# shivangchopra11/MedMoE

Measured on AMD Instinct MI355X. Metric: image-text pairs/sec at global batch 1024, higher is better.
Workload: dtype bf16; 1 GPU; cfg2: ViT-B/16 + 12-layer text tower (frozen), 8 experts top-2, 224x224x3 + 77 tokens, fwd+bwd+clip+Adam; global_batch=1024, per_gpu_batch=1024, parallelism=dp1

## Files before the change

### medmoe_amd/csrc/attention.hip

```cpp
#include "common.h"
#include "options.h"

#define HD 64

__device__ __forceinline__ int tpos(int r) {
  const int o = r & 31;
  return (r & ~31) + (((o & 15) >> 2) << 3) + ((o >> 4) << 2) + (o & 3);
}

template <int CNT, int RT>
__device__ __forceinline__ void fill_rowmajor(char* lds, const bf16_t* src, long long row_stride, int n_valid, int tid) {
  constexpr int PER = (CNT + RT - 1) / RT;
  uint4 v[PER];
#pragma unroll
  for (int i = 0; i < PER; ++i) {
    const int idx = min(tid + i * RT, CNT - 1);
    const int row = idx >> 3, c = idx & 7;
    v[i] = *(const uint4*)(src + (long long)min(row, n_valid - 1) * row_stride + c * 8);
  }
#pragma unroll
  for (int i = 0; i < PER; ++i) {
    const int idx = tid + i * RT;
    const int row = idx >> 3, c = idx & 7;
    if (idx < CNT) *(uint4*)(lds + row * 128 + ((c ^ (row & 7)) << 4)) = v[i];
  }
}

__device__ __forceinline__ void fill_transposed(char* lds, const bf16_t* src, long long row_stride, int n_valid,
                                                int stride_bytes, int tid) {
  for (int i = tid; i < (64 * stride_bytes) / 16; i += 256) *(uint4*)(lds + i * 16) = make_uint4(0, 0, 0, 0);
  __syncthreads();
  for (int idx = tid; idx < n_valid * 8; idx += 256) {
    const int row = idx >> 3, c = idx & 7;
    const uint4 v = *(const uint4*)(src + (long long)row * row_stride + c * 8);
    const uint32_t w[4] = {v.x, v.y, v.z, v.w};
    const int pos = tpos(row);
#pragma unroll
    for (int e = 0; e < 4; ++e) {
      *(bf16_t*)(lds + (c * 8 + 2 * e) * stride_bytes + pos * 2) = (bf16_t)(w[e] & 0xffff);
      *(bf16_t*)(lds + (c * 8 + 2 * e + 1) * stride_bytes + pos * 2) = (bf16_t)(w[e] >> 16);
    }
  }
}

__device__ __forceinline__ bf16x8_t tr_frag(const char* img, int row0, int col0, int lane) {
  const int q = (lane & 15) >> 2, pp = lane & 3;
  const int ra = row0 + 4 * (lane >> 4) + q, rb = ra + 16;
  const int col = col0 + 4 * pp;
  const int ch = col >> 3, within = (col & 7) << 1;
  const bf16x4_t lo = __builtin_amdgcn_ds_read_tr16_b64_v4bf16(
      (__attribute__((address_space(3))) bf16x4_t*)(img + ra * 128 + ((ch ^ (ra & 7)) << 4) + within));
  const bf16x4_t hi = __builtin_amdgcn_ds_read_tr16_b64_v4bf16(
      (__attribute__((address_space(3))) bf16x4_t*)(img + rb * 128 + ((ch ^ (rb & 7)) << 4) + within));
  return __builtin_shufflevector(lo, hi, 0, 1, 2, 3, 4, 5, 6, 7);
}

__device__ __forceinline__ bf16x8_t load_frag_global(const bf16_t* base, long long row_stride, int row, int chunk) {
  const uint4 v = *(const uint4*)(base + (long long)row * row_stride + chunk * 8);
  return __builtin_bit_cast(bf16x8_t, v);
}

__device__ __forceinline__ bf16x8_t pack_frag(const f32x4_t& a, const f32x4_t& b) {
  uint4 v;
  v.x = pack2bf(a[0], a[1]); v.y = pack2bf(a[2], a[3]);
  v.z = pack2bf(b[0], b[1]); v.w = pack2bf(b[2], b[3]);
  return __builtin_bit_cast(bf16x8_t, v);
}

template <int NKT>
struct AttnGeom {
  static constexpr int NKP = NKT * 16;
  static constexpr int KS = (NKT + 1) / 2;
  static constexpr int RMROWS = KS * 32;
  static constexpr int RM_BYTES = RMROWS * 128;
  static constexpr int FILL = RMROWS * 8;
};

#ifdef ATTN_TIMING
__device__ unsigned long long g_attn_timing[8];
#define ATTN_T(...) __VA_ARGS__
#else
#define ATTN_T(...)
#endif

template <int NKT, bool MASKED, int RT>
__global__ __launch_bounds__(RT, RT == 256 ? 2 : 4) void attn_fwd_kernel(const bf16_t* __restrict__ qkv, bf16_t* __restrict__ out,
                                                         float* __restrict__ lse, const unsigned char* __restrict__ key_mask,
                                                         int Nmax, int H, float scale, const int* __restrict__ seq_off) {
  using G = AttnGeom<NKT>;
  constexpr int CH = 8;
  constexpr int NCH = (NKT + CH - 1) / CH;
  __shared__ __attribute__((aligned(16))) char smem[2 * G::RM_BYTES + G::NKP * 4];
  char* sK = smem;
  char* sV = smem + G::RM_BYTES;
  float* sMask = (float*)(smem + 2 * G::RM_BYTES);
  const int tid = threadIdx.x, lane = tid & 63, wid = tid >> 6;
  const int b = blockIdx.x / H, h = blockIdx.x - b * H;
  const int D = H * HD;
  const long long rs = 3LL * D;
  const long long row0 = seq_off ? (long long)seq_off[b] : (long long)b * Nmax;
  const int N = seq_off ? max(1, min(seq_off[b + 1] - seq_off[b], Nmax)) : Nmax;
  const bf16_t* base = qkv + row0 * rs + h * HD;

  fill_rowmajor<G::FILL, RT>(sK, base + D, rs, N, tid);
  fill_rowmajor<G::FILL, RT>(sV, base + 2 * D, rs, N, tid);
  for (int k = tid; k < G::NKP; k += RT)
    sMask[k] = (k < N && (!key_mask || key_mask[(long long)b * Nmax + k])) ? 0.f : -INFINITY;
  __syncthreads();

  const int fr = lane & 15, g = lane >> 4;
  const int nqb = (N + 15) >> 4;
  const float c2 = scale * 1.44269504088896f;
  bf16x8_t qf[2], qn[2];
  {
    const int qc0 = min(wid * 16 + fr, N - 1);
    qf[0] = load_frag_global(base, rs, qc0, g);
    qf[1] = load_frag_global(base, rs, qc0, 4 + g);
  }
  for (int qb = wid; qb < nqb; qb += RT / 64) {
    const int q = qb * 16 + fr;
    {
      const int qcn = min((qb + RT / 64) * 16 + fr, N - 1);
      qn[0] = load_frag_global(base, rs, qcn, g);
      qn[1] = load_frag_global(base, rs, qcn, 4 + g);
    }
    float m = -INFINITY, lp = 0.f;
    f32x4_t o[4];
#pragma unroll
    for (int nd = 0; nd < 4; ++nd) o[nd] = (f32x4_t){0.f, 0.f, 0.f, 0.f};
#pragma unroll 1
    for (int c = 0; c < NCH; ++c) {
      const int kt0 = c * CH;
      f32x4_t s[CH];
#pragma unroll
      for (int u = 0; u < CH; ++u) {
        s[u] = (f32x4_t){0.f, 0.f, 0.f, 0.f};
        if (kt0 + u < NKT) {
          const char* kr = sK + ((kt0 + u) * 16 + fr) * 128;
#pragma unroll
          for (int ks = 0; ks < 2; ++ks) {
            const bf16x8_t kf = *(const bf16x8_t*)(kr + (((ks * 4 + g) ^ (fr & 7)) << 4));
            s[u] = __builtin_amdgcn_mfma_f32_16x16x32_bf16(kf, qf[ks], s[u], 0, 0, 0);
          }
        }
      }
      float alpha;
      f32x2_t l2 = {0.f, 0.f};
      if constexpr (MASKED) {
        float bm = -INFINITY;
#pragma unroll
        for (int u = 0; u < CH; ++u)
          if (kt0 + u < NKT) {
            const float4 mk = *(const float4*)(sMask + (kt0 + u) * 16 + g * 4);
            const f32x2_t t0 = (f32x2_t){s[u][0], s[u][1]} * c2 + (f32x2_t){mk.x, mk.y};
            const f32x2_t t1 = (f32x2_t){s[u][2], s[u][3]} * c2 + (f32x2_t){mk.z, mk.w};
            s[u][0] = t0[0]; s[u][1] = t0[1]; s[u][2] = t1[0]; s[u][3] = t1[1];
            bm = fmaxf(fmaxf(bm, fmaxf(t0[0], t0[1])), fmaxf(t1[0], t1[1]));
          }
        bm = fmaxf(bm, __shfl_xor(bm, 16, 64));
        bm = fmaxf(bm, __shfl_xor(bm, 32, 64));
        const float mn = fmaxf(m, bm);
        const float ms = (mn == -INFINITY) ? 0.f : mn;
        alpha = __builtin_amdgcn_exp2f(m - ms);
        m = mn;
#pragma unroll
        for (int u = 0; u < CH; ++u)
          if (kt0 + u < NKT) {
            const f32x2_t d0 = (f32x2_t){s[u][0], s[u][1]} - ms, d1 = (f32x2_t){s[u][2], s[u][3]} - ms;
            const f32x2_t e0 = {__builtin_amdgcn_exp2f(d0[0]), __builtin_amdgcn_exp2f(d0[1])};
            const f32x2_t e1 = {__builtin_amdgcn_exp2f(d1[0]), __builtin_amdgcn_exp2f(d1[1])};
            s[u][0] = e0[0]; s[u][1] = e0[1]; s[u][2] = e1[0]; s[u][3] = e1[1];
            l2 += e0 + e1;
          }
      } else {
        float bm = fmaxf(fmaxf(s[0][0], s[0][1]), fmaxf(s[0][2], s[0][3]));
#pragma unroll
        for (int u = 1; u < CH; ++u)
          if (kt0 + u < NKT) bm = fmaxf(fmaxf(bm, fmaxf(s[u][0], s[u][1])), fmaxf(s[u][2], s[u][3]));
        bm = fmaxf(bm, __shfl_xor(bm, 16, 64));
        bm = fmaxf(bm, __shfl_xor(bm, 32, 64));
        const float mn = fmaxf(m, bm * c2);
        alpha = __builtin_amdgcn_exp2f(m - mn);
        m = mn;
        const float nm = -mn;
#pragma unroll
        for (int u = 0; u < CH; ++u)
          if (kt0 + u < NKT) {
            const f32x2_t d0 = (f32x2_t){s[u][0], s[u][1]} * c2 + nm, d1 = (f32x2_t){s[u][2], s[u][3]} * c2 + nm;
            f32x2_t e0 = {__builtin_amdgcn_exp2f(d0[0]), __builtin_amdgcn_exp2f(d0[1])};
            f32x2_t e1 = {__builtin_amdgcn_exp2f(d1[0]), __builtin_amdgcn_exp2f(d1[1])};
            if ((kt0 + u) * 16 + 16 > N) {
              const int k0 = (kt0 + u) * 16 + g * 4;
              e0[0] = k0 < N ? e0[0] : 0.f; e0[1] = k0 + 1 < N ? e0[1] : 0.f;
              e1[0] = k0 + 2 < N ? e1[0] : 0.f; e1[1] = k0 + 3 < N ? e1[1] : 0.f;
            }
            s[u][0] = e0[0]; s[u][1] = e0[1]; s[u][2] = e1[0]; s[u][3] = e1[1];
            l2 += e0 + e1;
          }
      }
      lp = lp * alpha + l2[0] + l2[1];
#pragma unroll
      for (int nd = 0; nd < 4; ++nd) {
        if (c > 0) o[nd] *= alpha;
#pragma unroll
        for (int t = 0; t < CH / 2; ++t)
          if (kt0 + 2 * t < NKT) {
            const bf16x8_t pf = pack_frag(s[2 * t], s[2 * t + 1]);
            const bf16x8_t vf = tr_frag(sV, (kt0 + 2 * t) * 16, nd * 16, lane);
            o[nd] = __builtin_amdgcn_mfma_f32_16x16x32_bf16(vf, pf, o[nd], 0, 0, 0);
          }
      }
    }
    float l = lp;
    l += __shfl_xor(l, 16, 64);
    l += __shfl_xor(l, 32, 64);
    const float inv = l > 0.f ? 1.f / l : 0.f;
    if (q < N) {
      if (g == 0) lse[((long long)b * H + h) * Nmax + q] = (m + __log2f(l)) * 0.693147180559945f;
#pragma unroll
      for (int nd = 0; nd < 4; ++nd) {
        const f32x4_t v = o[nd] * inv;
        uint2 pk; pk.x = pack2bf(v[0], v[1]); pk.y = pack2bf(v[2], v[3]);
        *(uint2*)(out + (row0 + q) * D + h * HD + nd * 16 + g * 4) = pk;
      }
    }
    qf[0] = qn[0]; qf[1] = qn[1];
  }
}

template <int NKT, bool MASKED, int RT>
__global__ __launch_bounds__(RT, 4) void attn_bwd_dq_kernel(const bf16_t* __restrict__ qkv, const bf16_t* __restrict__ o,
                                                          const bf16_t* __restrict__ dout, const float* __restrict__ lse,
                                                          const unsigned char* __restrict__ key_mask,
                                                          bf16_t* __restrict__ dqkv, float* __restrict__ delta,
                                                          int Nmax, int H, float scale, const int* __restrict__ seq_off) {
  using G = AttnGeom<NKT>;
  __shared__ __attribute__((aligned(16))) char smem[2 * G::RM_BYTES + G::NKP * 4];
  char* sK = smem;
  char* sV = smem + G::RM_BYTES;
  float* sMask = (float*)(smem + 2 * G::RM_BYTES);
  const int tid = threadIdx.x, lane = tid & 63, wid = tid >> 6;
  const int b = blockIdx.x / H, h = blockIdx.x - b * H;
  const int D = H * HD;
  const long long rs = 3LL * D;
  const long long row0 = seq_off ? (long long)seq_off[b] : (long long)b * Nmax;
  const int N = seq_off ? max(1, min(seq_off[b + 1] - seq_off[b], Nmax)) : Nmax;
  const bf16_t* base = qkv + row0 * rs + h * HD;
  const bf16_t* obase = o + row0 * D + h * HD;
  const bf16_t* dobase = dout + row0 * D + h * HD;

  fill_rowmajor<G::FILL, RT>(sK, base + D, rs, N, tid);
  fill_rowmajor<G::FILL, RT>(sV, base + 2 * D, rs, N, tid);
  for (int k = tid; k < G::NKP; k += RT)
    sMask[k] = (k < N && (!key_mask || key_mask[(long long)b * Nmax + k])) ? 0.f : -INFINITY;
  __syncthreads();

  const int fr = lane & 15, g = lane >> 4;
  const int nqb = (N + 15) >> 4;
  bf16x8_t qf[2], dof[2], of[2], qn[2], don[2], on[2];
  {
    const int qc0 = min(wid * 16 + fr, N - 1);
#pragma unroll
    for (int ks = 0; ks < 2; ++ks) {
      qf[ks] = load_frag_global(base, rs, qc0, ks * 4 + g);
      dof[ks] = load_frag_global(dobase, D, qc0, ks * 4 + g);
      of[ks] = load_frag_global(obase, D, qc0, ks * 4 + g);
    }
  }
  for (int qb = wid; qb < nqb; qb += RT / 64) {
    const int q = qb * 16 + fr;
    const int qc = min(q, N - 1);
    {
      const int qcn = min((qb + RT / 64) * 16 + fr, N - 1);
#pragma unroll
      for (int ks = 0; ks < 2; ++ks) {
        qn[ks] = load_frag_global(base, rs, qcn, ks * 4 + g);
        don[ks] = load_frag_global(dobase, D, qcn, ks * 4 + g);
        on[ks] = load_frag_global(obase, D, qcn, ks * 4 + g);
      }
    }
    float dl = 0.f;
#pragma unroll
    for (int ks = 0; ks < 2; ++ks)
#pragma unroll
      for (int e = 0; e < 8; ++e) dl += (float)dof[ks][e] * (float)of[ks][e];
    dl += __shfl_xor(dl, 16, 64);
    dl += __shfl_xor(dl, 32, 64);
    const float c2 = scale * 1.44269504088896f;
    const float nL2 = -lse[((long long)b * H + h) * Nmax + qc] * 1.44269504088896f;
    if (g == 0 && q < N) delta[((long long)b * H + h) * Nmax + q] = dl;

    f32x4_t acc[4];
#pragma unroll
    for (int nd = 0; nd < 4; ++nd) acc[nd] = (f32x4_t){0.f, 0.f, 0.f, 0.f};
#pragma unroll 1
    for (int t = 0; t < G::KS; ++t) {
      f32x4_t ds[2];
#pragma unroll
      for (int u = 0; u < 2; ++u) {
        const int kt = 2 * t + u;
        ds[u] = (f32x4_t){0.f, 0.f, 0.f, 0.f};
        if (kt < NKT) {
          f32x4_t s = {0.f, 0.f, 0.f, 0.f}, dp = {0.f, 0.f, 0.f, 0.f};
          const char* kr = sK + (kt * 16 + fr) * 128;
          const char* vr = sV + (kt * 16 + fr) * 128;
#pragma unroll
          for (int ks = 0; ks < 2; ++ks) {
            const int off = ((ks * 4 + g) ^ (fr & 7)) << 4;
            s = __builtin_amdgcn_mfma_f32_16x16x32_bf16(*(const bf16x8_t*)(kr + off), qf[ks], s, 0, 0, 0);
            dp = __builtin_amdgcn_mfma_f32_16x16x32_bf16(*(const bf16x8_t*)(vr + off), dof[ks], dp, 0, 0, 0);
          }
          if (MASKED || kt * 16 + 16 > N) {
            const float4 mk = *(const float4*)(sMask + kt * 16 + g * 4);
            const float mkv[4] = {mk.x, mk.y, mk.z, mk.w};
#pragma unroll
            for (int r = 0; r < 4; ++r) ds[u][r] = __builtin_amdgcn_exp2f(s[r] * c2 + (mkv[r] + nL2)) * (dp[r] - dl);
          } else {
            const f32x2_t t0 = (f32x2_t){s[0], s[1]} * c2 + nL2, t1 = (f32x2_t){s[2], s[3]} * c2 + nL2;
            const f32x2_t g0 = (f32x2_t){dp[0], dp[1]} - dl, g1 = (f32x2_t){dp[2], dp[3]} - dl;
            const f32x2_t d0 = (f32x2_t){__builtin_amdgcn_exp2f(t0[0]), __builtin_amdgcn_exp2f(t0[1])} * g0;
            const f32x2_t d1 = (f32x2_t){__builtin_amdgcn_exp2f(t1[0]), __builtin_amdgcn_exp2f(t1[1])} * g1;
            ds[u] = (f32x4_t){d0[0], d0[1], d1[0], d1[1]};
          }
        }
      }
      const bf16x8_t dsf = pack_frag(ds[0], ds[1]);
#pragma unroll
      for (int nd = 0; nd < 4; ++nd) {
        const bf16x8_t ktf = tr_frag(sK, t * 32, nd * 16, lane);
        acc[nd] = __builtin_amdgcn_mfma_f32_16x16x32_bf16(ktf, dsf, acc[nd], 0, 0, 0);
      }
    }
    if (q < N) {
#pragma unroll
      for (int nd = 0; nd < 4; ++nd) {
        const f32x4_t v = acc[nd] * scale;
        uint2 pk; pk.x = pack2bf(v[0], v[1]); pk.y = pack2bf(v[2], v[3]);
        *(uint2*)(dqkv + (row0 + q) * rs + h * HD + nd * 16 + g * 4) = pk;
      }
    }
#pragma unroll
    for (int ks = 0; ks < 2; ++ks) { qf[ks] = qn[ks]; dof[ks] = don[ks]; of[ks] = on[ks]; }
  }
}

template <int NKT, int RT>
__global__ __launch_bounds__(RT, 4) void attn_bwd_dkv_kernel(const bf16_t* __restrict__ qkv, const bf16_t* __restrict__ dout,
                                                           const float* __restrict__ lse, const float* __restrict__ delta,
                                                           const unsigned char* __restrict__ key_mask,
                                                           bf16_t* __restrict__ dqkv, int Nmax, int H, float scale,
                                                           const int* __restrict__ seq_off) {
  using G = AttnGeom<NKT>;
  __shared__ __attribute__((aligned(16))) char smem[2 * G::RM_BYTES + G::NKP * 12];
  char* sQ = smem;
  char* sDO = smem + G::RM_BYTES;
  float* sMask = (float*)(smem + 2 * G::RM_BYTES);
  float* sLse = sMask + G::NKP;
  float* sDelta = sLse + G::NKP;
  const int tid = threadIdx.x, lane = tid & 63, wid = tid >> 6;
  const int b = blockIdx.x / H, h = blockIdx.x - b * H;
  const int D = H * HD;
  const long long rs = 3LL * D;
  const long long row0 = seq_off ? (long long)seq_off[b] : (long long)b * Nmax;
  const int N = seq_off ? max(1, min(seq_off[b + 1] - seq_off[b], Nmax)) : Nmax;
  const bf16_t* base = qkv + row0 * rs + h * HD;
  const bf16_t* dobase = dout + row0 * D + h * HD;

  fill_rowmajor<G::FILL, RT>(sQ, base, rs, N, tid);
  fill_rowmajor<G::FILL, RT>(sDO, dobase, D, N, tid);
  for (int k = tid; k < G::NKP; k += RT) {
    const bool valid = k < N;
    sMask[k] = (valid && (!key_mask || key_mask[(long long)b * Nmax + k])) ? 0.f : -INFINITY;
    sLse[k] = valid ? lse[((long long)b * H + h) * Nmax + k] * 1.44269504088896f : INFINITY;
    sDelta[k] = valid ? delta[((long long)b * H + h) * Nmax + k] : 0.f;
  }
  __syncthreads();

  const int fr = lane & 15, g = lane >> 4;
  const int nkb = (N + 15) >> 4;
  bf16x8_t kf[2], vf[2], kn[2], vn[2];
  {
    const int kc0 = min(wid * 16 + fr, N - 1);
#pragma unroll
    for (int ks = 0; ks < 2; ++ks) {
      kf[ks] = load_frag_global(base + D, rs, kc0, ks * 4 + g);
      vf[ks] = load_frag_global(base + 2 * D, rs, kc0, ks * 4 + g);
    }
  }
  for (int kb = wid; kb < nkb; kb += RT / 64) {
    const int key = kb * 16 + fr;
    {
      const int kcn = min((kb + RT / 64) * 16 + fr, N - 1);
#pragma unroll
      for (int ks = 0; ks < 2; ++ks) {
        kn[ks] = load_frag_global(base + D, rs, kcn, ks * 4 + g);
        vn[ks] = load_frag_global(base + 2 * D, rs, kcn, ks * 4 + g);
      }
    }
    const float mk = sMask[kb * 16 + fr];
    const float c2 = scale * 1.44269504088896f;
    f32x4_t dk[4], dv[4];
#pragma unroll
    for (int nd = 0; nd < 4; ++nd) { dk[nd] = (f32x4_t){0.f, 0.f, 0.f, 0.f}; dv[nd] = (f32x4_t){0.f, 0.f, 0.f, 0.f}; }

#pragma unroll 1
    for (int t = 0; t < G::KS; ++t) {
      f32x4_t pp[2], dss[2];
#pragma unroll
      for (int u = 0; u < 2; ++u) {
        const int qt = 2 * t + u;
        if (qt < NKT) {
          f32x4_t s = {0.f, 0.f, 0.f, 0.f}, dp = {0.f, 0.f, 0.f, 0.f};
          const char* qr = sQ + (qt * 16 + fr) * 128;
          const char* dr = sDO + (qt * 16 + fr) * 128;
#pragma unroll
          for (int ks = 0; ks < 2; ++ks) {
            const int off = ((ks * 4 + g) ^ (fr & 7)) << 4;
            s = __builtin_amdgcn_mfma_f32_16x16x32_bf16(*(const bf16x8_t*)(qr + off), kf[ks], s, 0, 0, 0);
            dp = __builtin_amdgcn_mfma_f32_16x16x32_bf16(*(const bf16x8_t*)(dr + off), vf[ks], dp, 0, 0, 0);
          }
          const float4 L4 = *(const float4*)(sLse + qt * 16 + g * 4);
          const float4 D4 = *(const float4*)(sDelta + qt * 16 + g * 4);
          const float Lv[4] = {L4.x, L4.y, L4.z, L4.w}, Dv[4] = {D4.x, D4.y, D4.z, D4.w};
          const f32x2_t t0 = (f32x2_t){s[0], s[1]} * c2 + (mk - (f32x2_t){Lv[0], Lv[1]});
          const f32x2_t t1 = (f32x2_t){s[2], s[3]} * c2 + (mk - (f32x2_t){Lv[2], Lv[3]});
          const f32x2_t p0 = {__builtin_amdgcn_exp2f(t0[0]), __builtin_amdgcn_exp2f(t0[1])};
          const f32x2_t p1 = {__builtin_amdgcn_exp2f(t1[0]), __builtin_amdgcn_exp2f(t1[1])};
          const f32x2_t d0 = p0 * ((f32x2_t){dp[0], dp[1]} - (f32x2_t){Dv[0], Dv[1]});
          const f32x2_t d1 = p1 * ((f32x2_t){dp[2], dp[3]} - (f32x2_t){Dv[2], Dv[3]});
          pp[u] = (f32x4_t){p0[0], p0[1], p1[0], p1[1]};
          dss[u] = (f32x4_t){d0[0], d0[1], d1[0], d1[1]};
        } else {
          pp[u] = (f32x4_t){0.f, 0.f, 0.f, 0.f};
          dss[u] = (f32x4_t){0.f, 0.f, 0.f, 0.f};
        }
      }
      const bf16x8_t pf = pack_frag(pp[0], pp[1]);
      const bf16x8_t dsf = pack_frag(dss[0], dss[1]);
#pragma unroll
      for (int nd = 0; nd < 4; ++nd) {
        const bf16x8_t dot = tr_frag(sDO, t * 32, nd * 16, lane);
        const bf16x8_t qt_ = tr_frag(sQ, t * 32, nd * 16, lane);
        dv[nd] = __builtin_amdgcn_mfma_f32_16x16x32_bf16(dot, pf, dv[nd], 0, 0, 0);
        dk[nd] = __builtin_amdgcn_mfma_f32_16x16x32_bf16(qt_, dsf, dk[nd], 0, 0, 0);
      }
    }
    if (key < N) {
      bf16_t* row = dqkv + (row0 + key) * rs + h * HD;
#pragma unroll
      for (int nd = 0; nd < 4; ++nd) {
        const f32x4_t kv = dk[nd] * scale;
        uint2 pk; pk.x = pack2bf(kv[0], kv[1]); pk.y = pack2bf(kv[2], kv[3]);
        *(uint2*)(row + D + nd * 16 + g * 4) = pk;
        pk.x = pack2bf(dv[nd][0], dv[nd][1]); pk.y = pack2bf(dv[nd][2], dv[nd][3]);
        *(uint2*)(row + 2 * D + nd * 16 + g * 4) = pk;
      }
    }
#pragma unroll
    for (int ks = 0; ks < 2; ++ks) { kf[ks] = kn[ks]; vf[ks] = vn[ks]; }
  }
}

#define SB 64
#define SB_BYTES (SB * 128)

__device__ __forceinline__ void stage_load(uint4 (&v)[2], const bf16_t* src, long long row_stride, int row0, int n_valid, int tid) {
#pragma unroll
  for (int i = 0; i < 2; ++i) {
    const int idx = tid + i * 256;
    const int row = idx >> 3, c = idx & 7;
    v[i] = *(const uint4*)(src + (long long)min(row0 + row, n_valid - 1) * row_stride + c * 8);
  }
}
__device__ __forceinline__ void stage_store(char* lds, const uint4 (&v)[2], int tid) {
#pragma unroll
  for (int i = 0; i < 2; ++i) {
    const int idx = tid + i * 256;
    const int row = idx >> 3, c = idx & 7;
    *(uint4*)(lds + row * 128 + ((c ^ (row & 7)) << 4)) = v[i];
  }
}
__device__ __forceinline__ bf16x8_t rm_frag(const char* img, int t16, int ks, int fr, int g) {
  return *(const bf16x8_t*)(img + (t16 * 16 + fr) * 128 + (((ks * 4 + g) ^ (fr & 7)) << 4));
}

template <bool MASKED>
__global__ __launch_bounds__(256) void attn_fwd_stream_kernel(const bf16_t* __restrict__ qkv, bf16_t* __restrict__ out,
                                                              float* __restrict__ lse, const unsigned char* __restrict__ key_mask,
                                                              int N, int H, int QB, float scale) {
  __shared__ __attribute__((aligned(16))) char smem[4 * SB_BYTES + 2 * SB * 4];
  const int tid = threadIdx.x, lane = tid & 63, wid = tid >> 6;
  const int fr = lane & 15, g = lane >> 4;
  const int id = xcd_remap(blockIdx.x, gridDim.x);
  const int bh = id / QB, qc = id - bh * QB;
  const int b = bh / H, h = bh - b * H;
  const int D = H * HD;
  const long long rs = 3LL * D;
  const bf16_t* base = qkv + (long long)b * N * rs + h * HD;
  const int q0 = qc * 64 + wid * 16;
  const bool active = q0 < N;
  const int q = q0 + fr;
  bf16x8_t qf[2];
  {
    const int qr = min(q, N - 1);
    qf[0] = load_frag_global(base, rs, qr, g);
    qf[1] = load_frag_global(base, rs, qr, 4 + g);
  }
  const int nkb = (N + SB - 1) / SB;
  auto bufK = [&](int i) { return smem + i * 2 * SB_BYTES; };
  auto bufV = [&](int i) { return smem + i * 2 * SB_BYTES + SB_BYTES; };
  float* sMaskAll = (float*)(smem + 4 * SB_BYTES);
  auto mask_of = [&](int key) -> float { return (key < N && (!key_mask || key_mask[(long long)b * N + key])) ? 0.f : -INFINITY; };
  uint4 kr[2], vr[2];
  stage_load(kr, base + D, rs, 0, N, tid);
  stage_load(vr, base + 2 * D, rs, 0, N, tid);
  stage_store(bufK(0), kr, tid); stage_store(bufV(0), vr, tid);
  if (tid < SB) sMaskAll[tid] = mask_of(tid);
  __syncthreads();

  const float c2 = scale * 1.44269504088896f;
  float m = -INFINITY, lp = 0.f;
  f32x4_t o[4];
#pragma unroll
  for (int nd = 0; nd < 4; ++nd) o[nd] = (f32x4_t){0.f, 0.f, 0.f, 0.f};
  for (int kb = 0; kb < nkb; ++kb) {
    const int cur = kb & 1;
    const bool more = kb + 1 < nkb;
    float mnext = 0.f;
    if (more) {
      stage_load(kr, base + D, rs, (kb + 1) * SB, N, tid);
      stage_load(vr, base + 2 * D, rs, (kb + 1) * SB, N, tid);
      if (tid < SB) mnext = mask_of((kb + 1) * SB + tid);
    }
    if (active) {
      const char* sK = bufK(cur);
      const char* sV = bufV(cur);
      const float* sM = sMaskAll + cur * SB;
      f32x4_t s[4];
#pragma unroll
      for (int kt = 0; kt < 4; ++kt) {
        s[kt] = (f32x4_t){0.f, 0.f, 0.f, 0.f};
#pragma unroll
        for (int ks = 0; ks < 2; ++ks) s[kt] = __builtin_amdgcn_mfma_f32_16x16x32_bf16(rm_frag(sK, kt, ks, fr, g), qf[ks], s[kt], 0, 0, 0);
      }
      float alpha;
      f32x2_t l2 = {0.f, 0.f};
      if constexpr (MASKED) {
        float bm = -INFINITY;
#pragma unroll
        for (int kt = 0; kt < 4; ++kt) {
          const float4 mk = *(const float4*)(sM + kt * 16 + g * 4);
          const f32x2_t t0 = (f32x2_t){s[kt][0], s[kt][1]} * c2 + (f32x2_t){mk.x, mk.y};
          const f32x2_t t1 = (f32x2_t){s[kt][2], s[kt][3]} * c2 + (f32x2_t){mk.z, mk.w};
          s[kt][0] = t0[0]; s[kt][1] = t0[1]; s[kt][2] = t1[0]; s[kt][3] = t1[1];
          bm = fmaxf(fmaxf(bm, fmaxf(t0[0], t0[1])), fmaxf(t1[0], t1[1]));
        }
        bm = fmaxf(bm, __shfl_xor(bm, 16, 64));
        bm = fmaxf(bm, __shfl_xor(bm, 32, 64));
        const float mn = fmaxf(m, bm);
        const float ms = (mn == -INFINITY) ? 0.f : mn;
        alpha = __builtin_amdgcn_exp2f(m - ms);
        m = mn;
#pragma unroll
        for (int kt = 0; kt < 4; ++kt) {
          const f32x2_t d0 = (f32x2_t){s[kt][0], s[kt][1]} - ms, d1 = (f32x2_t){s[kt][2], s[kt][3]} - ms;
          const f32x2_t e0 = {__builtin_amdgcn_exp2f(d0[0]), __builtin_amdgcn_exp2f(d0[1])};
          const f32x2_t e1 = {__builtin_amdgcn_exp2f(d1[0]), __builtin_amdgcn_exp2f(d1[1])};
          s[kt][0] = e0[0]; s[kt][1] = e0[1]; s[kt][2] = e1[0]; s[kt][3] = e1[1];
          l2 += e0 + e1;
        }
      } else {
        float bm = fmaxf(fmaxf(s[0][0], s[0][1]), fmaxf(s[0][2], s[0][3]));
#pragma unroll
        for (int kt = 1; kt < 4; ++kt) bm = fmaxf(fmaxf(bm, fmaxf(s[kt][0], s[kt][1])), fmaxf(s[kt][2], s[kt][3]));
        bm = fmaxf(bm, __shfl_xor(bm, 16, 64));
        bm = fmaxf(bm, __shfl_xor(bm, 32, 64));
        const float mn = fmaxf(m, bm * c2);
        alpha = __builtin_amdgcn_exp2f(m - mn);
        m = mn;
        const float nm = -mn;
        const bool tail = kb * SB + SB > N;
#pragma unroll
        for (int kt = 0; kt < 4; ++kt) {
          const f32x2_t d0 = (f32x2_t){s[kt][0], s[kt][1]} * c2 + nm, d1 = (f32x2_t){s[kt][2], s[kt][3]} * c2 + nm;
          f32x2_t e0 = {__builtin_amdgcn_exp2f(d0[0]), __builtin_amdgcn_exp2f(d0[1])};
          f32x2_t e1 = {__builtin_amdgcn_exp2f(d1[0]), __builtin_amdgcn_exp2f(d1[1])};
          if (tail) {
            const int k0 = kb * SB + kt * 16 + g * 4;
            e0[0] = k0 < N ? e0[0] : 0.f; e0[1] = k0 + 1 < N ? e0[1] : 0.f;
            e1[0] = k0 + 2 < N ? e1[0] : 0.f; e1[1] = k0 + 3 < N ? e1[1] : 0.f;
          }
          s[kt][0] = e0[0]; s[kt][1] = e0[1]; s[kt][2] = e1[0]; s[kt][3] = e1[1];
          l2 += e0 + e1;
        }
      }
      lp = lp * alpha + l2[0] + l2[1];
      bf16x8_t pf[2];
      pf[0] = pack_frag(s[0], s[1]);
      pf[1] = pack_frag(s[2], s[3]);
#pragma unroll
      for (int nd = 0; nd < 4; ++nd) {
        o[nd] *= alpha;
#pragma unroll
        for (int t = 0; t < 2; ++t) o[nd] = __builtin_amdgcn_mfma_f32_16x16x32_bf16(tr_frag(sV, t * 32, nd * 16, lane), pf[t], o[nd], 0, 0, 0);
      }
    }
    if (more) {
      stage_store(bufK(cur ^ 1), kr, tid); stage_store(bufV(cur ^ 1), vr, tid);
      if (tid < SB) sMaskAll[(cur ^ 1) * SB + tid] = mnext;
    }
    __syncthreads();
  }
  if (!active) return;
  float l = lp;
  l += __shfl_xor(l, 16, 64);
  l += __shfl_xor(l, 32, 64);
  const float inv = l > 0.f ? 1.f / l : 0.f;
  if (q < N) {
    if (g == 0) lse[((long long)b * H + h) * N + q] = (m + __log2f(l)) * 0.693147180559945f;
#pragma unroll
    for (int nd = 0; nd < 4; ++nd) {
      const f32x4_t v = o[nd] * inv;
      uint2 pk; pk.x = pack2bf(v[0], v[1]); pk.y = pack2bf(v[2], v[3]);
      *(uint2*)(out + ((long long)b * N + q) * D + h * HD + nd * 16 + g * 4) = pk;
    }
  }
}

template <bool MASKED>
__global__ __launch_bounds__(256) void attn_bwd_dq_stream_kernel(const bf16_t* __restrict__ qkv, const bf16_t* __restrict__ o,
                                                                 const bf16_t* __restrict__ dout, const float* __restrict__ lse,
                                                                 const unsigned char* __restrict__ key_mask,
                                                                 bf16_t* __restrict__ dqkv, float* __restrict__ delta,
                                                                 int N, int H, int QB, float scale) {
  __shared__ __attribute__((aligned(16))) char smem[4 * SB_BYTES + 2 * SB * 4];
  const int tid = threadIdx.x, lane = tid & 63, wid = tid >> 6;
  const int fr = lane & 15, g = lane >> 4;
  const int id = xcd_remap(blockIdx.x, gridDim.x);
  const int bh = id / QB, qc = id - bh * QB;
  const int b = bh / H, h = bh - b * H;
  const int D = H * HD;
  const long long rs = 3LL * D;
  const bf16_t* base = qkv + (long long)b * N * rs + h * HD;
  const bf16_t* obase = o + (long long)b * N * D + h * HD;
  const bf16_t* dobase = dout + (long long)b * N * D + h * HD;
  const int q0 = qc * 64 + wid * 16;
  const bool active = q0 < N;
  const int q = q0 + fr, qr = min(q, N - 1);
  bf16x8_t qf[2], dof[2];
  float dl = 0.f;
  {
    bf16x8_t of[2];
#pragma unroll
    for (int ks = 0; ks < 2; ++ks) {
      qf[ks] = load_frag_global(base, rs, qr, ks * 4 + g);
      dof[ks] = load_frag_global(dobase, D, qr, ks * 4 + g);
      of[ks] = load_frag_global(obase, D, qr, ks * 4 + g);
    }
#pragma unroll
    for (int ks = 0; ks < 2; ++ks)
#pragma unroll
      for (int e = 0; e < 8; ++e) dl += (float)dof[ks][e] * (float)of[ks][e];
    dl += __shfl_xor(dl, 16, 64);
    dl += __shfl_xor(dl, 32, 64);
  }
  const float c2 = scale * 1.44269504088896f;
  const float nL2 = -lse[((long long)b * H + h) * N + qr] * 1.44269504088896f;
  if (active && g == 0 && q < N) delta[((long long)b * H + h) * N + q] = dl;

  const int nkb = (N + SB - 1) / SB;
  auto bufK = [&](int i) { return smem + i * 2 * SB_BYTES; };
  auto bufV = [&](int i) { return smem + i * 2 * SB_BYTES + SB_BYTES; };
  float* sMaskAll = (float*)(smem + 4 * SB_BYTES);
  auto mask_of = [&](int key) -> float { return (key < N && (!key_mask || key_mask[(long long)b * N + key])) ? 0.f : -INFINITY; };
  uint4 kr[2], vr[2];
  stage_load(kr, base + D, rs, 0, N, tid);
  stage_load(vr, base + 2 * D, rs, 0, N, tid);
  stage_store(bufK(0), kr, tid); stage_store(bufV(0), vr, tid);
  if (tid < SB) sMaskAll[tid] = mask_of(tid);
  __syncthreads();
  f32x4_t acc[4];
#pragma unroll
  for (int nd = 0; nd < 4; ++nd) acc[nd] = (f32x4_t){0.f, 0.f, 0.f, 0.f};
  for (int kb = 0; kb < nkb; ++kb) {
    const int cur = kb & 1;
    const bool more = kb + 1 < nkb;
    float mnext = 0.f;
    if (more) {
      stage_load(kr, base + D, rs, (kb + 1) * SB, N, tid);
      stage_load(vr, base + 2 * D, rs, (kb + 1) * SB, N, tid);
      if (tid < SB) mnext = mask_of((kb + 1) * SB + tid);
    }
    if (active) {
      const char* sK = bufK(cur);
      const char* sV = bufV(cur);
      const float* sM = sMaskAll + cur * SB;
      f32x4_t ds[4];
#pragma unroll
      for (int kt = 0; kt < 4; ++kt) {
        f32x4_t s = {0.f, 0.f, 0.f, 0.f}, dp = {0.f, 0.f, 0.f, 0.f};
#pragma unroll
        for (int ks = 0; ks < 2; ++ks) {
          s = __builtin_amdgcn_mfma_f32_16x16x32_bf16(rm_frag(sK, kt, ks, fr, g), qf[ks], s, 0, 0, 0);
          dp = __builtin_amdgcn_mfma_f32_16x16x32_bf16(rm_frag(sV, kt, ks, fr, g), dof[ks], dp, 0, 0, 0);
        }
        if (MASKED || kb * SB + SB > N) {
          const float4 mk = *(const float4*)(sM + kt * 16 + g * 4);
          const float mkv[4] = {mk.x, mk.y, mk.z, mk.w};
#pragma unroll
          for (int r = 0; r < 4; ++r) ds[kt][r] = __builtin_amdgcn_exp2f(s[r] * c2 + (mkv[r] + nL2)) * (dp[r] - dl);
        } else {
          const f32x2_t t0 = (f32x2_t){s[0], s[1]} * c2 + nL2, t1 = (f32x2_t){s[2], s[3]} * c2 + nL2;
          const f32x2_t d0 = (f32x2_t){__builtin_amdgcn_exp2f(t0[0]), __builtin_amdgcn_exp2f(t0[1])} * ((f32x2_t){dp[0], dp[1]} - dl);
          const f32x2_t d1 = (f32x2_t){__builtin_amdgcn_exp2f(t1[0]), __builtin_amdgcn_exp2f(t1[1])} * ((f32x2_t){dp[2], dp[3]} - dl);
          ds[kt] = (f32x4_t){d0[0], d0[1], d1[0], d1[1]};
        }
      }
      const bf16x8_t dsf0 = pack_frag(ds[0], ds[1]), dsf1 = pack_frag(ds[2], ds[3]);
#pragma unroll
      for (int nd = 0; nd < 4; ++nd) {
        acc[nd] = __builtin_amdgcn_mfma_f32_16x16x32_bf16(tr_frag(sK, 0, nd * 16, lane), dsf0, acc[nd], 0, 0, 0);
        acc[nd] = __builtin_amdgcn_mfma_f32_16x16x32_bf16(tr_frag(sK, 32, nd * 16, lane), dsf1, acc[nd], 0, 0, 0);
      }
    }
    if (more) {
      stage_store(bufK(cur ^ 1), kr, tid); stage_store(bufV(cur ^ 1), vr, tid);
      if (tid < SB) sMaskAll[(cur ^ 1) * SB + tid] = mnext;
    }
    __syncthreads();
  }
  if (active && q < N) {
#pragma unroll
    for (int nd = 0; nd < 4; ++nd) {
      const f32x4_t v = acc[nd] * scale;
      uint2 pk; pk.x = pack2bf(v[0], v[1]); pk.y = pack2bf(v[2], v[3]);
      *(uint2*)(dqkv + ((long long)b * N + q) * rs + h * HD + nd * 16 + g * 4) = pk;
    }
  }
}

__global__ __launch_bounds__(256) void attn_bwd_dkv_stream_kernel(const bf16_t* __restrict__ qkv, const bf16_t* __restrict__ dout,
                                                                  const float* __restrict__ lse, const float* __restrict__ delta,
                                                                  const unsigned char* __restrict__ key_mask,
                                                                  bf16_t* __restrict__ dqkv, int N, int H, int QB, float scale) {
  __shared__ __attribute__((aligned(16))) char smem[4 * SB_BYTES + 4 * SB * 4];
  const int tid = threadIdx.x, lane = tid & 63, wid = tid >> 6;
  const int fr = lane & 15, g = lane >> 4;
  const int id = xcd_remap(blockIdx.x, gridDim.x);
  const int bh = id / QB, kc = id - bh * QB;
  const int b = bh / H, h = bh - b * H;
  const int D = H * HD;
  const long long rs = 3LL * D;
  const bf16_t* base = qkv + (long long)b * N * rs + h * HD;
  const bf16_t* dobase = dout + (long long)b * N * D + h * HD;
  const float* lrow = lse + ((long long)b * H + h) * N;
  const float* drow = delta + ((long long)b * H + h) * N;
  const int k0 = kc * 64 + wid * 16;
  const bool active = k0 < N;
  const int key = k0 + fr, kr_ = min(key, N - 1);
// ... 184 lines not shown
```

Baseline: 4781 pairs/s.

## Overlap attention LDS fill with fragment prefetch and widen output stores

The forward, dQ and dK/dV attention kernels now split their LDS staging into an issue phase and a commit phase, so the global loads for K/V (or Q/dO), the mask, LSE and delta, and the first Q/K fragments are all in flight before anything is written to shared memory. The dQ kernel also prefetches the next row's LSE alongside the other next-iteration fragments. Output and gradient tiles are repacked across lane groups with permlane16_swap so each lane issues 16-byte stores instead of 8-byte ones. Empty asm pins and fences keep the compiler from reordering the loads. The cost is higher register pressure from the extra live values, and the kernels now require one mask entry per thread.

```diff
diff --git a/medmoe_amd/csrc/attention.hip b/medmoe_amd/csrc/attention.hip
--- a/medmoe_amd/csrc/attention.hip
+++ b/medmoe_amd/csrc/attention.hip
@@ -1,5 +1,6 @@
 #include "common.h"
 #include "options.h"
+#include "attn_fill.h"
 
 #define HD 64
 
@@ -8,23 +9,38 @@
   return (r & ~31) + (((o & 15) >> 2) << 3) + ((o >> 4) << 2) + (o & 3);
 }
 
+typedef __attribute__((ext_vector_type(4))) unsigned attn_u32x4_t;
+
+template <typename T>
+__device__ __forceinline__ void attn_pin(T& v) { asm volatile("" : "+v"(v)); }
+
+__device__ __forceinline__ void attn_issue_fence() { asm volatile("" ::: "memory"); }
+
+__device__ __forceinline__ unsigned mask_byte_load(const unsigned char* key_mask, long long idx, const void* readable) {
+  const unsigned char* p = key_mask ? key_mask + idx : (const unsigned char*)readable;
+  return *p;
+}
+
 template <int CNT, int RT>
-__device__ __forceinline__ void fill_rowmajor(char* lds, const bf16_t* src, long long row_stride, int n_valid, int tid) {
-  constexpr int PER = (CNT + RT - 1) / RT;
-  uint4 v[PER];
-#pragma unroll
-  for (int i = 0; i < PER; ++i) {
-    const int idx = min(tid + i * RT, CNT - 1);
-    const int row = idx >> 3, c = idx & 7;
-    v[i] = *(const uint4*)(src + (long long)min(row, n_valid - 1) * row_stride + c * 8);
-  }
-#pragma unroll
-  for (int i = 0; i < PER; ++i) {
-    const int idx = tid + i * RT;
-    const int row = idx >> 3, c = idx & 7;
-    if (idx < CNT) *(uint4*)(lds + row * 128 + ((c ^ (row & 7)) << 4)) = v[i];
-  }
-}
+struct RmStage {
+  static constexpr int PER = attn_fill_per(CNT, RT);
+  attn_u32x4_t v[PER];
+  __device__ __forceinline__ void issue(const bf16_t* src, long long row_stride, int n_valid, int tid) {
+#pragma unroll
+    for (int i = 0; i < PER; ++i) {
+      const AttnPiece p = attn_fill_piece(CNT, RT, tid, i, n_valid);
+      v[i] = *(const attn_u32x4_t*)(src + (long long)p.src_row * row_stride + p.chunk * 8);
+    }
+  }
+  __device__ __forceinline__ void commit(char* lds, int tid) {
+#pragma unroll
+    for (int i = 0; i < PER; ++i) {
+      const AttnPiece p = attn_fill_piece(CNT, RT, tid, i, 1);
+      attn_pin(v[i]);
+      *(attn_u32x4_t*)(lds + p.slot) = v[i];
+    }
+  }
+};
 
 __device__ __forceinline__ void fill_transposed(char* lds, const bf16_t* src, long long row_stride, int n_valid,
                                                 int stride_bytes, int tid) {
@@ -66,6 +82,13 @@
   v.z = pack2bf(b[0], b[1]); v.w = pack2bf(b[2], b[3]);
   return __builtin_bit_cast(bf16x8_t, v);
 }
+
+__device__ __forceinline__ uint4 pair16(uint2 a, uint2 b) {
+  const auto x = __builtin_amdgcn_permlane16_swap(a.x, b.x, false, false);
+  const auto y = __builtin_amdgcn_permlane16_swap(a.y, b.y, false, false);
+  return make_uint4(x[0], y[0], x[1], y[1]);
+}
+__device__ __forceinline__ int pair16_col(int k, int g) { return (k + (g & 1)) * 16 + (g >> 1) * 8; }
 
 template <int NKT>
 struct AttnGeom {
@@ -102,27 +125,35 @@
   const int N = seq_off ? max(1, min(seq_off[b + 1] - seq_off[b], Nmax)) : Nmax;
   const bf16_t* base = qkv + row0 * rs + h * HD;
 
-  fill_rowmajor<G::FILL, RT>(sK, base + D, rs, N, tid);
-  fill_rowmajor<G::FILL, RT>(sV, base + 2 * D, rs, N, tid);
-  for (int k = tid; k < G::NKP; k += RT)
-    sMask[k] = (k < N && (!key_mask || key_mask[(long long)b * Nmax + k])) ? 0.f : -INFINITY;
-  __syncthreads();
-
+  static_assert(G::NKP <= RT, "one mask entry per thread");
   const int fr = lane & 15, g = lane >> 4;
   const int nqb = (N + 15) >> 4;
   const float c2 = scale * 1.44269504088896f;
   bf16x8_t qf[2], qn[2];
+  ATTN_T(const long long t_in = clock64();)
+  RmStage<G::FILL, RT> stK, stV;
+  stK.issue(base + D, rs, N, tid);
+  stV.issue(base + 2 * D, rs, N, tid);
+  unsigned mkb = mask_byte_load(key_mask, (long long)b * Nmax + min(tid, N - 1), base);
   {
     const int qc0 = min(wid * 16 + fr, N - 1);
     qf[0] = load_frag_global(base, rs, qc0, g);
     qf[1] = load_frag_global(base, rs, qc0, 4 + g);
   }
+  stK.commit(sK, tid);
+  stV.commit(sV, tid);
+  attn_pin(mkb);
+  if (tid < G::NKP) sMask[tid] = (tid < N && (!key_mask || mkb)) ? 0.f : -INFINITY;
+  attn_pin(qf[0]); attn_pin(qf[1]);
+  __syncthreads();
+  ATTN_T(const long long t_fill = clock64();)
   for (int qb = wid; qb < nqb; qb += RT / 64) {
     const int q = qb * 16 + fr;
     {
       const int qcn = min((qb + RT / 64) * 16 + fr, N - 1);
       qn[0] = load_frag_global(base, rs, qcn, g);
       qn[1] = load_frag_global(base, rs, qcn, 4 + g);
+      attn_issue_fence();
     }
     float m = -INFINITY, lp = 0.f;
     f32x4_t o[4];
@@ -215,17 +246,23 @@
     l += __shfl_xor(l, 16, 64);
     l += __shfl_xor(l, 32, 64);
     const float inv = l > 0.f ? 1.f / l : 0.f;
+    attn_pin(qn[0]); attn_pin(qn[1]);
+    uint2 pk[4];
+#pragma unroll
+    for (int nd = 0; nd < 4; ++nd) {
+      const f32x4_t v = o[nd] * inv;
+      pk[nd].x = pack2bf(v[0], v[1]); pk[nd].y = pack2bf(v[2], v[3]);
+    }
+    const uint4 w0 = pair16(pk[0], pk[1]), w1 = pair16(pk[2], pk[3]);
     if (q < N) {
       if (g == 0) lse[((long long)b * H + h) * Nmax + q] = (m + __log2f(l)) * 0.693147180559945f;
-#pragma unroll
-      for (int nd = 0; nd < 4; ++nd) {
-        const f32x4_t v = o[nd] * inv;
-        uint2 pk; pk.x = pack2bf(v[0], v[1]); pk.y = pack2bf(v[2], v[3]);
-        *(uint2*)(out + (row0 + q) * D + h * HD + nd * 16 + g * 4) = pk;
-      }
+      bf16_t* orow = out + (row0 + q) * D + h * HD;
+      *(uint4*)(orow + pair16_col(0, g)) = w0;
+      *(uint4*)(orow + pair16_col(2, g)) = w1;
     }
     qf[0] = qn[0]; qf[1] = qn[1];
   }
+  ATTN_T(if (tid == 0) { atomicAdd(&g_attn_timing[0], (unsigned long long)(t_fill - t_in)); atomicAdd(&g_attn_timing[4], (unsigned long long)(clock64() - t_in)); atomicAdd(&g_attn_timing[5], 1ull); })
 }
 
 template <int NKT, bool MASKED, int RT>
@@ -249,15 +286,16 @@
   const bf16_t* obase = o + row0 * D + h * HD;
   const bf16_t* dobase = dout + row0 * D + h * HD;
 
-  fill_rowmajor<G::FILL, RT>(sK, base + D, rs, N, tid);
-  fill_rowmajor<G::FILL, RT>(sV, base + 2 * D, rs, N, tid);
-  for (int k = tid; k < G::NKP; k += RT)
-    sMask[k] = (k < N && (!key_mask || key_mask[(long long)b * Nmax + k])) ? 0.f : -INFINITY;
-  __syncthreads();
-
+  static_assert(G::NKP <= RT, "one mask entry per thread");
   const int fr = lane & 15, g = lane >> 4;
   const int nqb = (N + 15) >> 4;
+  const float* lrow = lse + ((long long)b * H + h) * Nmax;
   bf16x8_t qf[2], dof[2], of[2], qn[2], don[2], on[2];
+  float lc, ln;
+  RmStage<G::FILL, RT> stK, stV;
+  stK.issue(base + D, rs, N, tid);
+  stV.issue(base + 2 * D, rs, N, tid);
+  unsigned mkb = mask_byte_load(key_mask, (long long)b * Nmax + min(tid, N - 1), base);
   {
     const int qc0 = min(wid * 16 + fr, N - 1);
 #pragma unroll
@@ -266,10 +304,18 @@
       dof[ks] = load_frag_global(dobase, D, qc0, ks * 4 + g);
       of[ks] = load_frag_global(obase, D, qc0, ks * 4 + g);
     }
-  }
+    lc = lrow[qc0];
+  }
+  stK.commit(sK, tid);
+  stV.commit(sV, tid);
+  attn_pin(mkb);
+  if (tid < G::NKP) sMask[tid] = (tid < N && (!key_mask || mkb)) ? 0.f : -INFINITY;
+#pragma unroll
+  for (int ks = 0; ks < 2; ++ks) { attn_pin(qf[ks]); attn_pin(dof[ks]); attn_pin(of[ks]); }
+  attn_pin(lc);
+  __syncthreads();
   for (int qb = wid; qb < nqb; qb += RT / 64) {
     const int q = qb * 16 + fr;
-    const int qc = min(q, N - 1);
     {
       const int qcn = min((qb + RT / 64) * 16 + fr, N - 1);
 #pragma unroll
@@ -278,6 +324,8 @@
         don[ks] = load_frag_global(dobase, D, qcn, ks * 4 + g);
         on[ks] = load_frag_global(obase, D, qcn, ks * 4 + g);
       }
+      ln = lrow[qcn];
+      attn_issue_fence();
     }
     float dl = 0.f;
 #pragma unroll
@@ -287,8 +335,7 @@
     dl += __shfl_xor(dl, 16, 64);
     dl += __shfl_xor(dl, 32, 64);
     const float c2 = scale * 1.44269504088896f;
-    const float nL2 = -lse[((long long)b * H + h) * Nmax + qc] * 1.44269504088896f;
-    if (g == 0 && q < N) delta[((long long)b * H + h) * Nmax + q] = dl;
+    const float nL2 = -lc * 1.44269504088896f;
 
     f32x4_t acc[4];
 #pragma unroll
@@ -331,16 +378,25 @@
         acc[nd] = __builtin_amdgcn_mfma_f32_16x16x32_bf16(ktf, dsf, acc[nd], 0, 0, 0);
       }
     }
+#pragma unroll
+    for (int ks = 0; ks < 2; ++ks) { attn_pin(qn[ks]); attn_pin(don[ks]); attn_pin(on[ks]); }
+    attn_pin(ln);
+    uint2 pk[4];
+#pragma unroll
+    for (int nd = 0; nd < 4; ++nd) {
+      const f32x4_t v = acc[nd] * scale;
+      pk[nd].x = pack2bf(v[0], v[1]); pk[nd].y = pack2bf(v[2], v[3]);
+    }
+    const uint4 w0 = pair16(pk[0], pk[1]), w1 = pair16(pk[2], pk[3]);
     if (q < N) {
-#pragma unroll
-      for (int nd = 0; nd < 4; ++nd) {
-        const f32x4_t v = acc[nd] * scale;
-        uint2 pk; pk.x = pack2bf(v[0], v[1]); pk.y = pack2bf(v[2], v[3]);
-        *(uint2*)(dqkv + (row0 + q) * rs + h * HD + nd * 16 + g * 4) = pk;
-      }
+      if (g == 0) delta[((long long)b * H + h) * Nmax + q] = dl;
+      bf16_t* qrow = dqkv + (row0 + q) * rs + h * HD;
+      *(uint4*)(qrow + pair16_col(0, g)) = w0;
+      *(uint4*)(qrow + pair16_col(2, g)) = w1;
     }
 #pragma unroll
     for (int ks = 0; ks < 2; ++ks) { qf[ks] = qn[ks]; dof[ks] = don[ks]; of[ks] = on[ks]; }
+    lc = ln;
   }
 }
 
@@ -366,19 +422,17 @@
   const bf16_t* base = qkv + row0 * rs + h * HD;
   const bf16_t* dobase = dout + row0 * D + h * HD;
 
-  fill_rowmajor<G::FILL, RT>(sQ, base, rs, N, tid);
-  fill_rowmajor<G::FILL, RT>(sDO, dobase, D, N, tid);
-  for (int k = tid; k < G::NKP; k += RT) {
-    const bool valid = k < N;
-    sMask[k] = (valid && (!key_mask || key_mask[(long long)b * Nmax + k])) ? 0.f : -INFINITY;
-    sLse[k] = valid ? lse[((long long)b * H + h) * Nmax + k] * 1.44269504088896f : INFINITY;
-    sDelta[k] = valid ? delta[((long long)b * H + h) * Nmax + k] : 0.f;
-  }
-  __syncthreads();
-
+  static_assert(G::NKP <= RT, "one mask / lse / delta entry per thread");
   const int fr = lane & 15, g = lane >> 4;
   const int nkb = (N + 15) >> 4;
   bf16x8_t kf[2], vf[2], kn[2], vn[2];
+  RmStage<G::FILL, RT> stQ, stDO;
+  stQ.issue(base, rs, N, tid);
+  stDO.issue(dobase, D, N, tid);
+  const int kcl = min(tid, N - 1);
+  unsigned mkb = mask_byte_load(key_mask, (long long)b * Nmax + kcl, base);
+  float lv = lse[((long long)b * H + h) * Nmax + kcl];
+  float dlv = delta[((long long)b * H + h) * Nmax + kcl];
   {
     const int kc0 = min(wid * 16 + fr, N - 1);
 #pragma unroll
@@ -387,6 +441,18 @@
       vf[ks] = load_frag_global(base + 2 * D, rs, kc0, ks * 4 + g);
     }
   }
+  stQ.commit(sQ, tid);
+  stDO.commit(sDO, tid);
+  attn_pin(mkb); attn_pin(lv); attn_pin(dlv);
+  if (tid < G::NKP) {
+    const bool valid = tid < N;
+    sMask[tid] = (valid && (!key_mask || mkb)) ? 0.f : -INFINITY;
+    sLse[tid] = valid ? lv * 1.44269504088896f : INFINITY;
+    sDelta[tid] = valid ? dlv : 0.f;
+  }
+#pragma unroll
+  for (int ks = 0; ks < 2; ++ks) { attn_pin(kf[ks]); attn_pin(vf[ks]); }
+  __syncthreads();
   for (int kb = wid; kb < nkb; kb += RT / 64) {
     const int key = kb * 16 + fr;
     {
@@ -396,6 +462,7 @@
         kn[ks] = load_frag_global(base + D, rs, kcn, ks * 4 + g);
         vn[ks] = load_frag_global(base + 2 * D, rs, kcn, ks * 4 + g);
       }
+      attn_issue_fence();
     }
     const float mk = sMask[kb * 16 + fr];
     const float c2 = scale * 1.44269504088896f;
@@ -445,16 +512,22 @@
         dk[nd] = __builtin_amdgcn_mfma_f32_16x16x32_bf16(qt_, dsf, dk[nd], 0, 0, 0);
       }
     }
+#pragma unroll
+    for (int ks = 0; ks < 2; ++ks) { attn_pin(kn[ks]); attn_pin(vn[ks]); }
+    uint2 pkk[4], pkv[4];
+#pragma unroll
+    for (int nd = 0; nd < 4; ++nd) {
+      const f32x4_t kv = dk[nd] * scale;
+      pkk[nd].x = pack2bf(kv[0], kv[1]); pkk[nd].y = pack2bf(kv[2], kv[3]);
+      pkv[nd].x = pack2bf(dv[nd][0], dv[nd][1]); pkv[nd].y = pack2bf(dv[nd][2], dv[nd][3]);
+    }
+    const uint4 wk0 = pair16(pkk[0], pkk[1]), wk1 = pair16(pkk[2], pkk[3]), wv0 = pair16(pkv[0], pkv[1]), wv1 = pair16(pkv[2], pkv[3]);
     if (key < N) {
       bf16_t* row = dqkv + (row0 + key) * rs + h * HD;
-#pragma unroll
-      for (int nd = 0; nd < 4; ++nd) {
-        const f32x4_t kv = dk[nd] * scale;
-        uint2 pk; pk.x = pack2bf(kv[0], kv[1]); pk.y = pack2bf(kv[2], kv[3]);
-        *(uint2*)(row + D + nd * 16 + g * 4) = pk;
-        pk.x = pack2bf(dv[nd][0], dv[nd][1]); pk.y = pack2bf(dv[nd][2], dv[nd][3]);
-        *(uint2*)(row + 2 * D + nd * 16 + g * 4) = pk;
-      }
+      *(uint4*)(row + D + pair16_col(0, g)) = wk0;
+      *(uint4*)(row + D + pair16_col(2, g)) = wk1;
+      *(uint4*)(row + 2 * D + pair16_col(0, g)) = wv0;
+      *(uint4*)(row + 2 * D + pair16_col(2, g)) = wv1;
     }
 #pragma unroll
     for (int ks = 0; ks < 2; ++ks) { kf[ks] = kn[ks]; vf[ks] = vn[ks]; }
diff --git a/medmoe_amd/csrc/attn_fill.h b/medmoe_amd/csrc/attn_fill.h
--- /dev/null
+++ b/medmoe_amd/csrc/attn_fill.h
@@ -0,0 +1,28 @@
+#pragma once
+
+#if defined(__HIPCC__) || defined(__CUDACC__)
+#define ATTN_FILL_HD __host__ __device__ __forceinline__
+#else
+#define ATTN_FILL_HD inline
+#endif
+
+struct AttnPiece {
+  int row, chunk;
+  int slot;
+  int src_row;
+};
+
+ATTN_FILL_HD constexpr int attn_fill_per(int cnt, int rt) { return (cnt + rt - 1) / rt; }
+
+ATTN_FILL_HD AttnPiece attn_fill_piece(int cnt, int rt, int tid, int i, int n_valid) {
+  const int raw = tid + i * rt;
+  const int idx = raw < cnt - 1 ? raw : cnt - 1;
+  AttnPiece p;
+  p.row = idx >> 3;
+  p.chunk = idx & 7;
+  p.slot = p.row * 128 + ((p.chunk ^ (p.row & 7)) << 4);
+  p.src_row = p.row < n_valid - 1 ? p.row : n_valid - 1;
+  return p;
+}
+
+ATTN_FILL_HD constexpr int attn_rm_rows(int nkt) { return ((nkt + 1) / 2) * 32; }
```

Measured after the change: 4820 pairs/s, median of 6. No clear change (+0.8%).
